# NTU-CompHydroMet-Lab/P2I-GAN-benchmark

Measured on AMD Instinct MI355X. Metric: train frames/sec (128x128x16), higher is better.
Workload: dtype f32

## Files before the change

p2i-gan-benchmark_amd/csrc/conv_x6c.hip:

```cpp
#include "conv_common.h"

namespace p2i {

#ifdef P2I_STAMP
extern __device__ unsigned long long* p2i_stamp_buf;
#define X6C_NOW(v) do { __builtin_amdgcn_sched_barrier(0); asm volatile("s_memtime %0\n\ts_waitcnt lgkmcnt(0)" : "=s"(v) :: "memory"); __builtin_amdgcn_sched_barrier(0); } while (0)
#define X6C_ACC(sum, t_prev) do { unsigned long long t_; X6C_NOW(t_); sum += t_ - t_prev; t_prev = t_; } while (0)
#else
#define X6C_NOW(v) do { } while (0)
#define X6C_ACC(sum, t_prev) do { } while (0)
#endif

typedef __bf16 bf16x8c __attribute__((ext_vector_type(8)));
typedef unsigned u32x4c __attribute__((ext_vector_type(4)));

__device__ __forceinline__ unsigned pack_hi16c(float lo_elem, float hi_elem) {
  return __builtin_amdgcn_perm(__float_as_uint(hi_elem), __float_as_uint(lo_elem), 0x07060302u);
}
__device__ __forceinline__ float trunc_bf16c(float v) { return __uint_as_float(__float_as_uint(v) & 0xFFFF0000u); }
__device__ __forceinline__ void split8c(const float (&v)[8], u32x4c& hi, u32x4c& mid, u32x4c& lo) {
#pragma unroll
  for (int j = 0; j < 4; ++j) {
    const float a = v[2 * j], b = v[2 * j + 1];
    hi[j] = pack_hi16c(a, b);
    const float ra = a - trunc_bf16c(a), rb = b - trunc_bf16c(b);
    mid[j] = pack_hi16c(ra, rb);
    const float sa = ra - trunc_bf16c(ra), sb = rb - trunc_bf16c(rb);
    lo[j] = pack_hi16c(sa, sb);
  }
}

template <class S, class I>
__device__ __forceinline__ void split8_store(const float* __restrict__ p, S stride, u32x4c* __restrict__ out, I total, I i) {
  float v[8];
#pragma unroll
  for (int q = 0; q < 8; ++q) v[q] = p[(S)q * stride];
  u32x4c h, mi, lo;
  split8c(v, h, mi, lo);
  out[i] = h;
  out[total + i] = mi;
  out[2 * total + i] = lo;
}

__global__ __launch_bounds__(256) void wsplit_kernel(const float* __restrict__ wp, u32x4c* __restrict__ wb, int ntaps, int Ck, int CmPad) {
  const int KCt = Ck >> 3;
  const int total = ntaps * KCt * CmPad;
  for (int i = blockIdx.x * 256 + threadIdx.x; i < total; i += gridDim.x * 256) {
    const int m = i % CmPad;
    const int r = i / CmPad;
    const int kc = r % KCt, tap = r / KCt;
    const float* p = wp + ((size_t)tap * Ck + kc * 8) * CmPad + m;
    split8_store(p, (size_t)CmPad, wb, total, i);
  }
}

struct WsplitBatch { const float* wp[24]; u32x4c* wb[24]; int ntaps[24], Ck[24], CmPad[24]; };
__global__ __launch_bounds__(256) void wsplit_batched_kernel(const WsplitBatch b) {
  const int L = blockIdx.y;
  const float* wp = b.wp[L];
  u32x4c* wb = b.wb[L];
  const int Ck = b.Ck[L], CmPad = b.CmPad[L], KCt = Ck >> 3;
  const int total = b.ntaps[L] * KCt * CmPad;
  for (int i = blockIdx.x * 256 + threadIdx.x; i < total; i += gridDim.x * 256) {
    const int m = i % CmPad;
    const int r = i / CmPad;
    const int kc = r % KCt, tap = r / KCt;
    const float* p = wp + ((size_t)tap * Ck + kc * 8) * CmPad + m;
    split8_store(p, (size_t)CmPad, wb, total, i);
  }
}

__global__ __launch_bounds__(256) void split_planes_kernel(const float* __restrict__ x, u32x4c* __restrict__ planes, int B, int KCt, long long P) {
  const long long total = (long long)B * KCt * P;
  for (long long i = blockIdx.x * 256ll + threadIdx.x; i < total; i += (long long)gridDim.x * 256) {
    const long long pix = i % P, r = i / P;
    const float* px = x + (r * 8) * P + pix;
    split8_store(px, P, planes, total, i);
  }
}

X6Ctx& x6_ctx() {
  static thread_local X6Ctx c{nullptr, 0};
  return c;
}

int x6_split_weights(const float* wp, uint16_t* wb, int ntaps, int Ck, int CmPad, hipStream_t s) {
  const int total = ntaps * (Ck >> 3) * CmPad;
  const int blocks = total > 0 ? (total + 255) / 256 : 1;
  P2I_LAUNCH(wsplit_kernel, dim3(blocks > 2048 ? 2048 : blocks), dim3(256), 0, s, wp, reinterpret_cast<u32x4c*>(wb), ntaps, Ck, CmPad);
  return launch_status();
}

struct X6cGeom {
  const float* src; float* dst; const uint16_t* wb; const float* bias; const float* res; const float* mask_y;
  unsigned wb_bytes;
  int act_epi, mask_act;
  int B, Ck, Cm, CmPad;
  int sH, sW, dT, dH, dW, nH, nW;
  int ljb, ljh, ljw, eH, eW, CSl, bH, bW, nth, ntw;
  unsigned mg_ew, mg_eh;
  int ntaps_w, ksplit;
  int sT, nT, mT, oT, pT, ns, sdt0, sdt1, sdt2, swt0, swt1, swt2;
  int tap_off[9];
  int tap_w[9];
  int fused_atomic;
  int stagger;
  int vec4_epi;
  const u32x4c* splanes;
  unsigned plane_units;
  int cons_prio;
};

__device__ constexpr int X6C_CLS[9] = {3, 3, 3, 3, 2, 2, 1, 1, 0};

template <int NW> struct X6cTile {
  static constexpr int MAXCSL = NW == 8 ? 384 : 256;
  static constexpr int NI = (2 * MAXCSL + 64 * NW - 1) / (64 * NW);
};

#define X6C_WAIT1(b) asm volatile("s_waitcnt vmcnt(%0)" ::"n"(b) : "memory")
#define X6C_WAIT2(b) if (n < (b) + 1) { X6C_WAIT1(b); } else { X6C_WAIT1((b) + 1); }
#define X6C_WAIT4(b) if (n < (b) + 2) { X6C_WAIT2(b) } else { X6C_WAIT2((b) + 2) }
#define X6C_WAIT8(b) if (n < (b) + 4) { X6C_WAIT4(b) } else { X6C_WAIT4((b) + 4) }
#define X6C_WAIT16(b) if (n < (b) + 8) { X6C_WAIT8(b) } else { X6C_WAIT8((b) + 8) }
#define X6C_WAIT32(b) if (n < (b) + 16) { X6C_WAIT16(b) } else { X6C_WAIT16((b) + 16) }
__device__ __forceinline__ void x6c_wait_vm(int n) {
  if (n < 0 || n > 62) n = 0;
  if (n < 32) { X6C_WAIT32(0) } else { X6C_WAIT32(32) }
}

template <int NW, int TM, bool FUSED = false, int TPS = 3>
__global__ __launch_bounds__(64 * NW) void patch_gemm_x6c_kernel(const X6cGeom g) {
  constexpr int NCLS = FUSED ? 4 : 1;
  constexpr int NSTG = 9 / TPS;
  static_assert(TPS == 3 || TPS == 9, "taps per stage");
  extern __shared__ __attribute__((aligned(16))) float smem[];
#ifdef P2I_STAMP
  unsigned long long st_entry, st_prev, st_wait = 0, st_bar = 0, st_issue = 0, st_mfma = 0, st_loop0;
  X6C_NOW(st_entry);
#endif
  constexpr int MB = 32 * TM, NTHR = 64 * NW, NI = X6cTile<NW>::NI;
  constexpr int RING = TPS == 9 ? 3 : (TM == 2 ? 4 : 6), LEAD = RING - 1;
  constexpr int WST = 6 * TPS * MB;
  constexpr int NWI = WST / 64;
  const int CSl = g.CSl;
  int* ptab = reinterpret_cast<int*>(smem);
  const int ptab_sz = (CSl + 3) & ~3;
  u32x4c* wbuf = reinterpret_cast<u32x4c*>(smem + ptab_sz);
  u32x4c* planes = wbuf + RING * WST;
  const int PST = 6 * CSl;

  const int tid = threadIdx.x, lane = tid & 63, wave = __builtin_amdgcn_readfirstlane(tid >> 6);
  const int l31 = lane & 31, lhi = lane >> 5;
  int tile = blockIdx.x;
  const int tw = tile % g.ntw; tile /= g.ntw;
  const int th = tile % g.nth;
  const int tb = tile / g.nth;
  const int j0b = tb << g.ljb, j0h = th << g.ljh, j0w = tw << g.ljw;
  const int o0 = blockIdx.y * MB;
  const int JWm = (1 << g.ljw) - 1, JHm = (1 << g.ljh) - 1;
  const int sHW = g.sH * g.sW;
  const int src_h0 = j0h + g.bH, src_w0 = j0w + g.bW;
  const int KCt = g.Ck >> 3;
  const int cps = g.Ck >> 4;
  const int cs = g.sT * sHW;
  const int nimg = g.B * g.nT;
  const int c0 = blockIdx.z * ((g.ns * cps) / g.ksplit);

  for (int e = tid; e < CSl; e += NTHR) {
    const int row = fast_div(e, g.mg_ew);
    const int ew = e - row * g.eW;
    const int jb = fast_div(row, g.mg_eh);
    const int eh = row - jb * g.eH;
    const int n = j0b + jb, h = src_h0 + eh, w = src_w0 + ew;
    const int b = n / g.nT, lt = n - b * g.nT;
    ptab[e] = (n < nimg && (unsigned)h < (unsigned)g.sH && (unsigned)w < (unsigned)g.sW) ? ((b * g.Ck) * g.sT + lt * g.mT) * sHW + h * g.sW + w : -1;
  }
  const int pix = wave * 32 + l31;
  const int pjw = pix & JWm, pjh = (pix >> g.ljw) & JHm, pjb = pix >> (g.ljw + g.ljh);
  const int lane_base = (pjb * g.eH + pjh) * g.eW + pjw + lhi * CSl;
  int toff[9];
#pragma unroll
  for (int t = 0; t < 9; ++t) toff[t] = g.tap_off[t];

  f32x16 acc[NCLS][TM];
#pragma unroll
  for (int q = 0; q < NCLS; ++q)
#pragma unroll
    for (int i = 0; i < TM; ++i)
#pragma unroll
      for (int r = 0; r < 16; ++r) acc[q][i][r] = 0.f;

  const v4i32 rs_w = make_rsrc(g.wb, g.wb_bytes);
  const unsigned wbuf_la = lds_base(smem) + 4u * ptab_sz;
  const int wl_m = TM == 2 ? lane : l31, wl_kg = TM == 2 ? 0 : lhi;
  const int wvoff = (o0 + wl_m < g.CmPad) ? (wl_kg * g.CmPad + wl_m) * 16 : -16;
  __syncthreads();

  int it_off[NI], it_dst[NI], it_f0[NI];
#pragma unroll
  for (int it = 0; it < NI; ++it) {
    const int item = it * NTHR + tid;
    const int kg = item >= CSl ? 1 : 0, e = item - kg * CSl;
    const bool in = item < 2 * CSl;
    const int po = in ? ptab[e] : -1;
    it_off[it] = po < 0 ? -1 : po + kg * 8 * cs;
    it_dst[it] = in ? kg * CSl + e : -1;
    const int jbi = fast_div(fast_div(in ? e : 0, g.mg_ew), g.mg_eh);
    it_f0[it] = ((j0b + jbi) % g.nT) * g.mT;
  }
  float pv[NI][8];
// ... 150 lines not shown
        if constexpr (TPS == 9) {
          if (more_c && (t == 4 || t == 6 || t == 7) && t == split_t) {
            x6c_wait_vm(nwb(sa));
            __builtin_amdgcn_sched_barrier(0);
            split_patch(planes + ((c + 1) & 1) * PST);
            __builtin_amdgcn_sched_barrier(0);
          }
        }
        load_tap(wsl, pb, TPS * b + t + 1, (t + 1) % 3);
        mfma_tap(t % 3, TPS * b + t);
        ilv();
        __builtin_amdgcn_sched_barrier(0);
      }
      if (TPS == 3 && late) { staging(); __builtin_amdgcn_sched_barrier(0); }
      X6C_ACC(st_mfma, st_prev);
      {
        int n = 0;
#pragma unroll
        for (int j = 2; j <= LEAD; ++j) n += nwb(s + j);
        if constexpr (TPS == 3) {
#pragma unroll
          for (int j = 0; j <= LEAD - 2; ++j) {
            const int bj = ((b - j) % 3 + 3) % 3;
            if (bj == 0 && s - j >= 0 && (s - j) / 3 + 1 < nch) n += NPL;
          }
        }
        x6c_wait_vm(n);
      }
      asm volatile("s_waitcnt lgkmcnt(0)" ::: "memory");
      X6C_ACC(st_wait, st_prev);
      __builtin_amdgcn_s_barrier();
      X6C_ACC(st_bar, st_prev);
      if (s + 1 < nst) load_tap(wlane + ((s + 1) % RING) * WST, b == NSTG - 1 ? pbn : pb, b == NSTG - 1 ? 0 : TPS * b + TPS, 0);
      mfma_tap(2, TPS * b + TPS - 1);
      ilv();
      __builtin_amdgcn_sched_barrier(0);
      X6C_ACC(st_mfma, st_prev);
    }
  }
#ifdef P2I_STAMP
  unsigned long long st_loop_end; X6C_NOW(st_loop_end);
#endif

  const int gw = j0w + pjw, gh = j0h + pjh, gn = j0b + pjb;
  const bool pvld = gn < nimg && gh < g.nH && gw < g.nW;
  const int dHW = g.dT * g.dH * g.dW;
  const int gb_ = gn / g.nT, glt = gn - gb_ * g.nT;
  if constexpr (FUSED) {
    const size_t pos0 = (size_t)gb_ * g.Cm * dHW + (size_t)(glt * g.oT + g.pT) * g.dH * g.dW + (size_t)(2 * gh) * g.dW + 2 * gw;
#pragma unroll
    for (int ph = 0; ph < 2; ++ph)
#pragma unroll
      for (int i = 0; i < TM; ++i)
        epilogue_pair16(acc[2 * ph][i], acc[2 * ph + 1][i], o0 + i * 32, lhi, g.Cm, pvld, pos0 + (size_t)ph * g.dW, (size_t)dHW,
                        (g.fused_atomic && blockIdx.z) ? nullptr : g.res, g.mask_y, g.mask_act, g.dst, g.fused_atomic != 0);
  } else {
    const size_t pos = (size_t)gb_ * g.Cm * dHW + (size_t)(glt * g.oT + g.pT) * g.dH * g.dW + (size_t)gh * g.dW + gw;
#pragma unroll
    for (int i = 0; i < TM; ++i)
      if (g.ksplit > 1)
        epilogue_tile16(acc[0][i], o0 + i * 32, lhi, g.Cm, pvld, pos, (size_t)dHW, blockIdx.z ? nullptr : g.bias, P2I_ACT_NONE,
                        blockIdx.z ? nullptr : g.res, g.mask_y, g.mask_act, g.dst, true);
      else
        epilogue_tile16(acc[0][i], o0 + i * 32, lhi, g.Cm, pvld, pos, (size_t)dHW, g.bias, g.act_epi, g.res, g.mask_y, g.mask_act, g.dst);
  }
#ifdef P2I_STAMP
  if (p2i_stamp_buf && lane == 0) {
    asm volatile("s_waitcnt vmcnt(0)" ::: "memory");
    unsigned long long st_x; X6C_NOW(st_x);
    unsigned long long* o = p2i_stamp_buf + ((size_t)(blockIdx.x + gridDim.x * blockIdx.y) * NW + wave) * 8;
    o[0] = st_wait; o[1] = st_bar; o[2] = st_issue; o[3] = st_mfma; o[4] = st_loop_end - st_loop0; o[5] = st_loop0; o[6] = st_loop0 - st_entry;
    o[7] = st_x - st_loop_end;
  }
#endif
}


template <int TM, int TPS, bool FUSED = false, bool EPI4 = false, int NPW = 4, int TN = 2, bool PRE = false>
__global__ __launch_bounds__(64 * (4 + NPW)) void patch_gemm_x6p_kernel(const X6cGeom g) {
  constexpr int NSTG = 9 / TPS;
  constexpr int NCLS = FUSED ? 4 : 1;
  static_assert(TPS == 3 || TPS == 9, "taps per stage");
  extern __shared__ __attribute__((aligned(16))) float smem[];
  constexpr int MB = 32 * TM, NCW = 4, NTHR = 64 * (NCW + NPW), NPT = 64 * NPW;
  constexpr int NI = (2 * (TN == 2 ? X6cTile<8>::MAXCSL : X6cTile<4>::MAXCSL) + NPT - 1) / NPT;
  constexpr int RING = TPS == 9 ? 3 : (TM == 2 ? 4 : 6), LEAD = RING - 1;
  constexpr int WST = 6 * TPS * MB, NWI = WST / 64;
  const int CSl = g.CSl;
  int* ptab = reinterpret_cast<int*>(smem);
  const int ptab_sz = (CSl + 3) & ~3;
  u32x4c* wbuf = reinterpret_cast<u32x4c*>(smem + ptab_sz);
  u32x4c* planes = wbuf + RING * WST;
  const int PST = 6 * CSl;

  const int tid = threadIdx.x, lane = tid & 63, wave = __builtin_amdgcn_readfirstlane(tid >> 6);
  const int l31 = lane & 31, lhi = lane >> 5;
  int tile = blockIdx.x;
  const int tw = tile % g.ntw; tile /= g.ntw;
  const int th = tile % g.nth;
  const int tb = tile / g.nth;
  const int j0b = tb << g.ljb, j0h = th << g.ljh, j0w = tw << g.ljw;
  const int o0 = blockIdx.y * MB;
  const int JWm = (1 << g.ljw) - 1, JHm = (1 << g.ljh) - 1;
  const int sHW = g.sH * g.sW;
  const int src_h0 = j0h + g.bH, src_w0 = j0w + g.bW;
  const int KCt = g.Ck >> 3;
  const int cps = g.Ck >> 4;
  const int cs = g.sT * sHW;
  const int nimg = g.B * g.nT;
  const int c0 = blockIdx.z * ((g.ns * cps) / g.ksplit);
  const int nch = (g.ns * cps) / g.ksplit;
  const int nst = NSTG * nch;

  for (int e = tid; e < CSl; e += NTHR) {
    const int row = fast_div(e, g.mg_ew);
    const int ew = e - row * g.eW;
    const int jb = fast_div(row, g.mg_eh);
    const int eh = row - jb * g.eH;
    const int n = j0b + jb, h = src_h0 + eh, w = src_w0 + ew;
    const int b = n / g.nT, lt = n - b * g.nT;
    ptab[e] = (n < nimg && (unsigned)h < (unsigned)g.sH && (unsigned)w < (unsigned)g.sW) ? ((b * (PRE ? KCt : g.Ck)) * g.sT + lt * g.mT) * sHW + h * g.sW + w : -1;
  }
  __syncthreads();

#ifdef P2I_STAMP
  unsigned long long st_a = 0, st_b = 0, st_c = 0, st_d = 0, st_e = 0, st_f = 0, st_t0, st_t1, st_l0 = 0, st_l1 = 0, st_entry;
  X6C_NOW(st_entry);
#endif
  if (wave >= NCW) {
    const int ptid = tid - 64 * NCW, pw = wave - NCW;
    const v4i32 rs_w = make_rsrc(g.wb, g.wb_bytes);
    const unsigned wbuf_la = lds_base(smem) + 4u * ptab_sz;
    const int wl_m = TM == 2 ? lane : l31, wl_kg = TM == 2 ? 0 : lhi;
    const int wvoff = (o0 + wl_m < g.CmPad) ? (wl_kg * g.CmPad + wl_m) * 16 : -16;
    int it_off[NI], it_dst[NI], it_f0[NI];
#pragma unroll
    for (int it = 0; it < NI; ++it) {
      const int item = it * NPT + ptid;
      const int kg = item >= CSl ? 1 : 0, e = item - kg * CSl;
      const bool in = item < 2 * CSl;
      const int po = in ? ptab[e] : -1;
      it_off[it] = po < 0 ? -1 : po + kg * (PRE ? 1 : 8) * cs;
      it_dst[it] = in ? kg * CSl + e : -1;
      const int jbi = fast_div(fast_div(in ? e : 0, g.mg_ew), g.mg_eh);
      it_f0[it] = ((j0b + jbi) % g.nT) * g.mT;
    }
    float pv[PRE ? 1 : NI][8];
    u32x4c pq[PRE ? NI : 1][3];
    bool pok[NI];
    auto load_patch = [&](int c) {
      if constexpr (PRE) {
        const int cg = c0 + c;
        const int j = cg >= 2 * cps ? 2 : (cg >= cps ? 1 : 0);
        const int dt = j == 2 ? g.sdt2 : (j == 1 ? g.sdt1 : g.sdt0);
        int voff[NI];
#pragma unroll
        for (int it = 0; it < NI; ++it) {
          pok[it] = it_off[it] >= 0 && (unsigned)(it_f0[it] + dt) < (unsigned)g.sT;
          voff[it] = pok[it] ? (it_off[it] + dt * sHW) * 16 : 0;
        }
#pragma unroll
        for (int p = 0; p < 3; ++p) {
          const u32x4c* sq = g.splanes + (size_t)p * g.plane_units + (size_t)(cg - j * cps) * 2 * cs;
          const unsigned long long sq_u = (unsigned long long)__builtin_amdgcn_readfirstlane((int)(unsigned)(unsigned long long)sq) & 0xffffffffull;
          const unsigned long long sq_hi = (unsigned long long)(unsigned)__builtin_amdgcn_readfirstlane((int)((unsigned long long)sq >> 32));
          const unsigned long long sbase = sq_u | (sq_hi << 32);
#pragma unroll
          for (int it = 0; it < NI; ++it) {
            if (it == 0) asm volatile("s_nop 4\n\tglobal_load_dwordx4 %0, %1, %2" : "=v"(pq[it][p]) : "v"(voff[it]), "s"(sbase) : "memory");
            else asm volatile("global_load_dwordx4 %0, %1, %2" : "=v"(pq[it][p]) : "v"(voff[it]), "s"(sbase) : "memory");
          }
        }
      } else {
      const int cg = c0 + c;
      const int j = cg >= 2 * cps ? 2 : (cg >= cps ? 1 : 0);
      const int dt = j == 2 ? g.sdt2 : (j == 1 ? g.sdt1 : g.sdt0);
      const float* sc = g.src + (size_t)(cg - j * cps) * 16 * cs;
      int voff[NI];
#pragma unroll
      for (int it = 0; it < NI; ++it) {
        pok[it] = it_off[it] >= 0 && (unsigned)(it_f0[it] + dt) < (unsigned)g.sT;
        voff[it] = pok[it] ? (it_off[it] + dt * sHW) * 4 : 0;
      }
#pragma unroll
      for (int q = 0; q < 8; ++q) {
        const float* sq = sc + (size_t)q * cs;
        const unsigned long long sq_u = (unsigned long long)__builtin_amdgcn_readfirstlane((int)(unsigned)(unsigned long long)sq) & 0xffffffffull;
        const unsigned long long sq_hi = (unsigned long long)(unsigned)__builtin_amdgcn_readfirstlane((int)((unsigned long long)sq >> 32));
        const unsigned long long sbase = sq_u | (sq_hi << 32);
#pragma unroll
        for (int it = 0; it < NI; ++it) {
          if (it == 0) asm volatile("s_nop 4\n\tglobal_load_dword %0, %1, %2" : "=v"(pv[it][q]) : "v"(voff[it]), "s"(sbase) : "memory");
          else asm volatile("global_load_dword %0, %1, %2" : "=v"(pv[it][q]) : "v"(voff[it]), "s"(sbase) : "memory");
        }
      }
      }
    };
    auto split_patch = [&](u32x4c* pb) {
      if constexpr (PRE) {
#pragma unroll
        for (int it = 0; it < NI; ++it)
#pragma unroll
          for (int p = 0; p < 3; ++p) asm volatile("" : "+v"(pq[it][p]));
        const u32x4c zero = {0u, 0u, 0u, 0u};
#pragma unroll
        for (int it = 0; it < NI; ++it) {
          if (it_dst[it] < 0) continue;
          pb[it_dst[it]] = pok[it] ? pq[it][0] : zero;
          pb[2 * CSl + it_dst[it]] = pok[it] ? pq[it][1] : zero;
          pb[4 * CSl + it_dst[it]] = pok[it] ? pq[it][2] : zero;
        }
      } else {
#pragma unroll
      for (int it = 0; it < NI; ++it)
#pragma unroll
        for (int q = 0; q < 8; ++q) asm volatile("" : "+v"(pv[it][q]));
#pragma unroll
      for (int it = 0; it < NI; ++it) {
        if (it_dst[it] < 0) continue;
        float v[8];
#pragma unroll
        for (int q = 0; q < 8; ++q) v[q] = pok[it] ? pv[it][q] : 0.f;
        u32x4c h, mi, lo;
        split8c(v, h, mi, lo);
        pb[it_dst[it]] = h;
        pb[2 * CSl + it_dst[it]] = mi;
        pb[4 * CSl + it_dst[it]] = lo;
      }
      }
    };
    constexpr int NWR = (NWI + NPW - 1) / NPW;
    int w_soff[NWR][NSTG];
    unsigned w_dst[NWR];
#pragma unroll
    for (int r = 0; r < NWR; ++r) {
      const int u = pw + NPW * r;
      const int pt = TM == 2 ? u >> 1 : u, kg = TM == 2 ? u & 1 : 0;
      const int p = pt / TPS, tl = pt % TPS;
#pragma unroll
      for (int b = 0; b < NSTG; ++b)
        w_soff[r][b] = u < NWI ? __builtin_amdgcn_readfirstlane((((p * g.ntaps_w + g.tap_w[TPS * b + tl]) * KCt + kg) * g.CmPad + o0) * 16) : 0;
      w_dst[r] = wbuf_la + 16u * (unsigned)(u * 64);
    }
    const int w_cstep = 2 * g.CmPad * 16;
    const int w_tstep = KCt * g.CmPad * 16;
    auto issue_w = [&](int c, int b, int sb) {
      const int cg = c0 + c;
      const int j = cg >= 2 * cps ? 2 : (cg >= cps ? 1 : 0);
      const int soff = (cg - j * cps) * w_cstep + (j == 2 ? g.swt2 : (j == 1 ? g.swt1 : g.swt0)) * w_tstep;
#pragma unroll
      for (int r = 0; r < NWR; ++r)
        if (pw + NPW * r < NWI) dma_b128(rs_w, w_dst[r] + 16u * (unsigned)(sb * WST), wvoff, w_soff[r][b] + soff);
    };
    const int nw_mine = (NWI / NPW) + (pw < NWI % NPW ? 1 : 0);
    constexpr int NPL = (PRE ? 3 : 8) * NI;
    auto nwb = [&](int st) { return (st >= LEAD && st < nst) ? nw_mine : 0; };
    load_patch(0);
    {
      int n = 0;
#pragma unroll
      for (int st = 0; st < LEAD; ++st) n += nwb(st);
      x6c_wait_vm(n);
      __builtin_amdgcn_sched_barrier(0);
      split_patch(planes);
      if constexpr (TPS == 9) {
        if (nch > 1) load_patch(1);
        x6c_wait_vm(n - nwb(0) + (nch > 1 ? NPL : 0));
      } else {
        x6c_wait_vm(n - nwb(0));
      }
    }
    asm volatile("s_waitcnt lgkmcnt(0)" ::: "memory");
    __builtin_amdgcn_s_barrier();
    int s = 0;
    for (int c = 0; c < nch; ++c) {
      const bool more_c = c + 1 < nch;
#pragma unroll
      for (int b = 0; b < NSTG; ++b, ++s) {
        const int sa = s + LEAD;
        if constexpr (TPS == 9) {
#ifdef P2I_STAMP
          X6C_NOW(st_t0);
          if (s == 0) st_l0 = st_t0;
#endif
          if (more_c) {
            x6c_wait_vm(s == 0 ? 0 : nwb(s - 1 + LEAD));
            X6C_ACC(st_a, st_t0);
            __builtin_amdgcn_sched_barrier(0);
            split_patch(planes + ((c + 1) & 1) * PST);
            __builtin_amdgcn_sched_barrier(0);
            X6C_ACC(st_b, st_t0);
            if (c + 2 < nch) load_patch(c + 2);
            X6C_ACC(st_e, st_t0);
          }
          if (sa < nst) issue_w(c + LEAD, 0, sa % RING);
          X6C_ACC(st_f, st_t0);
          x6c_wait_vm(nwb(s + 2) + ((more_c && c + 2 < nch) ? NPL : 0));
          X6C_ACC(st_c, st_t0);
        } else {
          if (b == 0 && more_c) load_patch(c + 1);
          if (sa < nst) issue_w(c + (b + LEAD) / NSTG, (b + LEAD) % NSTG, sa % RING);
          if (b == NSTG - 1 && more_c) {
            int n = 0;
#pragma unroll
            for (int j = 0; j < NSTG; ++j) n += nwb(sa - j);
            x6c_wait_vm(n);
            __builtin_amdgcn_sched_barrier(0);
            split_patch(planes + ((c + 1) & 1) * PST);
          }
          int n = 0;
#pragma unroll
          for (int j = 2; j <= LEAD; ++j) n += nwb(s + j);
#pragma unroll
          for (int j = 0; j <= LEAD - 2; ++j) {
            const int sj = s - j;
            if (sj >= 0 && sj % NSTG == 0 && sj / NSTG + 1 < nch) n += NPL;
          }
          x6c_wait_vm(n);
        }
        asm volatile("s_waitcnt lgkmcnt(0)" ::: "memory");
#ifdef P2I_STAMP
        X6C_NOW(st_t1);
#endif
        __builtin_amdgcn_s_barrier();
#ifdef P2I_STAMP
        X6C_ACC(st_d, st_t1);
        st_l1 = st_t1;
#endif
      }
    }
  }

  const bool producer = wave >= NCW;
  const int cw = wave & (NCW - 1);
  int lane_base[TN], pjw_[TN], pjh_[TN], pjb_[TN];
#pragma unroll
  for (int nb = 0; nb < TN; ++nb) {
    const int pix = cw * 32 * TN + nb * 32 + l31;
    pjw_[nb] = pix & JWm; pjh_[nb] = (pix >> g.ljw) & JHm; pjb_[nb] = pix >> (g.ljw + g.ljh);
    lane_base[nb] = (pjb_[nb] * g.eH + pjh_[nb]) * g.eW + pjw_[nb] + lhi * CSl;
  }
  int toff[9];
#pragma unroll
  for (int t = 0; t < 9; ++t) toff[t] = g.tap_off[t];
  f32x16 acc[NCLS][TM][TN];
#pragma unroll
  for (int q = 0; q < NCLS; ++q)
#pragma unroll
    for (int i = 0; i < TM; ++i)
#pragma unroll
      for (int nb = 0; nb < TN; ++nb)
#pragma unroll
        for (int r = 0; r < 16; ++r) acc[q][i][nb][r] = 0.f;
  constexpr int PA[6] = {2, 0, 1, 1, 0, 0};
  constexpr int PB[6] = {0, 2, 1, 0, 1, 0};
  u32x4c A[3][TM][3], Bv[3][TN][3];
  auto load_tap = [&](const u32x4c* wsl, const u32x4c* pbuf, int tap, int buf) {
    const int tl = tap % TPS;
    const int to = toff[tap];
#pragma unroll
    for (int p = 0; p < 3; ++p) {
#pragma unroll
      for (int i = 0; i < TM; ++i) A[buf][i][p] = wsl[((p * TPS + tl) * 2) * MB + 32 * i];
#pragma unroll
      for (int nb = 0; nb < TN; ++nb) Bv[buf][nb][p] = pbuf[lane_base[nb] + p * 2 * CSl + to];
    }
  };
  auto mfma_tap = [&](int buf, int slot) {
    const int cl = FUSED ? X6C_CLS[slot] : 0;
#pragma unroll
    for (int q = 0; q < 6; ++q)
#pragma unroll
      for (int i = 0; i < TM; ++i)
#pragma unroll
        for (int nb = 0; nb < TN; ++nb)
          acc[cl][i][nb] = __builtin_amdgcn_mfma_f32_32x32x16_bf16(__builtin_bit_cast(bf16x8c, A[buf][i][PA[q]]), __builtin_bit_cast(bf16x8c, Bv[buf][nb][PB[q]]),
                                                                   acc[cl][i][nb], 0, 0, 0);
  };
  auto ilv = [&]() {
    constexpr int NR = 3 * TM + 3 * TN, NM = 6 * TM * TN;
#pragma unroll
    for (int i = 0; i < NM; ++i) {
      __builtin_amdgcn_sched_group_barrier(0x008, 1, 0);
      if (i < NR) __builtin_amdgcn_sched_group_barrier(0x100, 1, 0);
    }
  };
  const int dHW = g.dT * g.dH * g.dW;
  const int mynb = (TN == 2 && producer) ? 1 : 0;
  const bool has_epi = wave < 2 * NCW;
  const bool split = FUSED ? g.fused_atomic != 0 : g.ksplit > 1;
  const float* const bias_q = (split && blockIdx.z) ? nullptr : g.bias;
  const float* const res_q = (split && blockIdx.z) ? nullptr : g.res;
  const bool blk1 = TN == 2 && producer;
  const int gw = j0w + (blk1 ? pjw_[TN - 1] : pjw_[0]), gh = j0h + (blk1 ? pjh_[TN - 1] : pjh_[0]), gn = j0b + (blk1 ? pjb_[TN - 1] : pjb_[0]);
  const bool pvld = gn < nimg && gh < g.nH && gw < g.nW;
  const int gb_ = gn / g.nT, glt = gn - gb_ * g.nT;
  const size_t img0 = (size_t)gb_ * g.Cm * dHW + (size_t)(glt * g.oT + g.pT) * g.dH * g.dW;
  const size_t pos0 = img0 + (size_t)(2 * gh) * g.dW + 2 * gw;
  const size_t pos = img0 + (size_t)gh * g.dW + gw;
  const int pg = cw * 32 * TN + mynb * 32 + 4 * (lane & 7);
  const int qw = pg & JWm, qh = (pg >> g.ljw) & JHm, qb = pg >> (g.ljw + g.ljh);
  const int hw = j0w + qw, hh = j0h + qh, hn = j0b + qb;
  const bool pv4 = hn < nimg && hh < g.nH && hw < g.nW;
  const int hb = hn / g.nT, hlt = hn - hb * g.nT;
  const size_t pos4 = (size_t)hb * g.Cm * dHW + (size_t)(hlt * g.oT + g.pT) * g.dH * g.dW + (size_t)hh * g.dW + hw;
  float* xch = reinterpret_cast<float*>(wbuf);
  float* tl = xch + 4 * NCLS * TM * 16 * 64 + wave * (32 * 36);
  EpiOps4p ops_p[FUSED ? 2 : 1];
  EpiOps4v ops_v[(!FUSED && EPI4) ? 2 : 1];
  EpiOps8 ops_t[(!FUSED && !EPI4) ? 2 : 1];
  auto fetch = [&](int slot, int k) {
    if constexpr (FUSED)
      epi_pair16_fetch(ops_p[slot], k & 3, o0 + ((k >> 2) % TM) * 32, lhi, g.Cm, pvld, pos0 + (size_t)(k / (4 * TM)) * g.dW, (size_t)dHW, res_q, g.mask_y);
    else if constexpr (EPI4)
      epi_tile16_v4_fetch(ops_v[slot], o0 + k * 32, lane, g.Cm, pos4, pv4, (size_t)dHW, bias_q, res_q, g.mask_y);
    else
      epi_tile16_fetch(ops_t[slot], k & 1, o0 + (k >> 1) * 32, lhi, g.Cm, pvld, pos, (size_t)dHW, bias_q, res_q, g.mask_y);
  };
  constexpr bool EARLY_C = !FUSED && TN == 1;
  const u32x4c* wlane = wbuf + lhi * MB + l31;
  if (!producer) {
    {
      const v4i32 rs_w = make_rsrc(g.wb, g.wb_bytes);
      const unsigned wbuf_la = lds_base(smem) + 4u * ptab_sz;
      const int wl_m = TM == 2 ? lane : l31, wl_kg = TM == 2 ? 0 : lhi;
      const int wvoff = (o0 + wl_m < g.CmPad) ? (wl_kg * g.CmPad + wl_m) * 16 : -16;
      const int w_cstep = 2 * g.CmPad * 16, w_tstep = KCt * g.CmPad * 16;
#pragma unroll
      for (int st = 0; st < LEAD; ++st) {
        if (st >= nst) break;
        const int cg = c0 + st / NSTG, b = st % NSTG;
        const int j = cg >= 2 * cps ? 2 : (cg >= cps ? 1 : 0);
        const int soff = (cg - j * cps) * w_cstep + (j == 2 ? g.swt2 : (j == 1 ? g.swt1 : g.swt0)) * w_tstep;
        for (int u = cw; u < NWI; u += NCW) {
          const int pt = TM == 2 ? u >> 1 : u, kg = TM == 2 ? u & 1 : 0;
          const int p = pt / TPS, tl = pt % TPS;
          const int so = (((p * g.ntaps_w + g.tap_w[TPS * b + tl]) * KCt + kg) * g.CmPad + o0) * 16 + soff;
          dma_b128(rs_w, wbuf_la + 16u * (unsigned)(u * 64 + (st % RING) * WST), wvoff, so);
        }
      }
      asm volatile("s_waitcnt vmcnt(0)" ::: "memory");
    }
    __builtin_amdgcn_s_barrier();
    if (g.cons_prio == 1) __builtin_amdgcn_s_setprio(1);
    else if (g.cons_prio == 2) __builtin_amdgcn_s_setprio(2);
    else if (g.cons_prio == 3) __builtin_amdgcn_s_setprio(3);
    load_tap(wlane, planes, 0, 0);
    int s = 0;
    for (int c = 0; c < nch; ++c) {
      const u32x4c* pb = planes + (c & 1) * PST;
      const u32x4c* pbn = planes + ((c + 1) & 1) * PST;
#pragma unroll
      for (int b = 0; b < NSTG; ++b, ++s) {
        const u32x4c* wsl = wlane + (s % RING) * WST;
        if constexpr (EARLY_C) { if (s + 1 == nst) fetch(0, 0); }
        __builtin_amdgcn_sched_barrier(0);
#pragma unroll
        for (int t = 0; t < TPS - 1; ++t) {
          load_tap(wsl, pb, TPS * b + t + 1, (t + 1) % 3);
          mfma_tap(t % 3, TPS * b + t);
          ilv();
          __builtin_amdgcn_sched_barrier(0);
        }
#ifdef P2I_STAMP
        X6C_NOW(st_t0);
        if (s == 0) st_l0 = st_t0;
#endif
        asm volatile("s_waitcnt lgkmcnt(0)" ::: "memory");
        X6C_ACC(st_a, st_t0);
        __builtin_amdgcn_s_barrier();
#ifdef P2I_STAMP
        X6C_ACC(st_d, st_t0);
        st_l1 = st_t0;
#endif
        if (s + 1 < nst) load_tap(wlane + ((s + 1) % RING) * WST, b == NSTG - 1 ? pbn : pb, b == NSTG - 1 ? 0 : TPS * b + TPS, 0);
        mfma_tap(2, TPS * b + TPS - 1);
        ilv();
        __builtin_amdgcn_sched_barrier(0);
      }
    }
  }
  if (!producer && g.cons_prio) __builtin_amdgcn_s_setprio(0);
  if (TN == 1 && producer) return;
  if (has_epi && !(EARLY_C && !producer)) fetch(0, 0);
  if constexpr (TN == 2) {
    if (!producer) {
#pragma unroll
      for (int q = 0; q < NCLS; ++q)
#pragma unroll
        for (int i = 0; i < TM; ++i)
#pragma unroll
          for (int r = 0; r < 16; ++r) xch[(((cw * NCLS + q) * TM + i) * 16 + r) * 64 + lane] = acc[q][i][1][r];
    }
    asm volatile("s_waitcnt lgkmcnt(0)" ::: "memory");
    __builtin_amdgcn_s_barrier();
    asm volatile("" ::: "memory");
    if (!has_epi) return;
    if (producer) {
#pragma unroll
      for (int q = 0; q < NCLS; ++q)
#pragma unroll
        for (int i = 0; i < TM; ++i)
#pragma unroll
          for (int r = 0; r < 16; ++r) acc[q][i][0][r] = xch[(((cw * NCLS + q) * TM + i) * 16 + r) * 64 + lane];
    }
  }
  if constexpr (FUSED) {
    auto finish = [&](int slot, int k) {
      const int ph = k / (4 * TM), i = (k >> 2) % TM;
      epi_pair16_finish(ops_p[slot], k & 3, acc[2 * ph][i][0], acc[2 * ph + 1][i][0], res_q, g.mask_y, g.mask_act, g.dst, split);
    };
    epilogue_pipelined<8 * TM>(fetch, finish, true);
  } else if constexpr (EPI4) {
    if (split) epilogue_pipelined<TM>(fetch, [&](int slot, int k) {
      epi_tile16_v4_finish(ops_v[slot], acc[0][k][0], tl, lane, P2I_ACT_NONE, res_q, g.mask_y, g.mask_act, g.dst, true); }, true);
    else epilogue_pipelined<TM>(fetch, [&](int slot, int k) {
      epi_tile16_v4_finish(ops_v[slot], acc[0][k][0], tl, lane, g.act_epi, g.res, g.mask_y, g.mask_act, g.dst, false); }, true);
  } else {
    if (split) epilogue_pipelined<2 * TM>(fetch, [&](int slot, int k) {
      epi_tile16_finish(ops_t[slot], k & 1, acc[0][k >> 1][0], bias_q, P2I_ACT_NONE, res_q, g.mask_y, g.mask_act, g.dst, true); }, true);
    else epilogue_pipelined<2 * TM>(fetch, [&](int slot, int k) {
      epi_tile16_finish(ops_t[slot], k & 1, acc[0][k >> 1][0], g.bias, g.act_epi, g.res, g.mask_y, g.mask_act, g.dst, false); }, true);
  }
#ifdef P2I_STAMP
  if (p2i_stamp_buf && lane == 0) {
    asm volatile("s_waitcnt vmcnt(0)" ::: "memory");
    unsigned long long st_end; X6C_NOW(st_end);
    unsigned long long* o = p2i_stamp_buf + ((size_t)(blockIdx.x + gridDim.x * blockIdx.y) * 8 + wave) * 8;
    o[0] = st_a; o[1] = st_d; o[2] = st_b; o[3] = st_c; o[4] = st_l1 - st_l0; o[5] = st_l0 - st_entry; o[6] = st_e; o[7] = st_end - st_l1;
  }
#endif
}

static bool x6c_on() { return P2I_ENV_ONCE("P2I_CONV_X6C", 1) != 0; }
static bool x6c_fused_on() { return P2I_ENV_ONCE("P2I_CONV_X6C_FUSED", 1) != 0; }
static int x6c_min_wg() { return env_int("P2I_X6C_MIN_WG", 200); }
static int x6c_min_wg_low() { return env_int("P2I_X6C_MIN_WG", env_int("P2I_X6C_MIN_WG_LOW", 64)); }
static int x6c_fused_min_wg() { return env_int("P2I_X6C_MIN_WG", 128); }
static int x6p_tn1() { return env_int("P2I_X6P_TN1", 1); }
static int x6c_forced() { return env_int("P2I_X6C_TILE", 0); }
static int x6c_stagger() { return env_int("P2I_X6C_STAGGER", 0); }
static int x6c_fused_ksplit() { return env_int("P2I_X6C_FUSED_KSPLIT", 0); }
static int x6p_npw() { return env_int("P2I_X6P_NPW", 8) == 4 ? 4 : 8; }
static int x6c_pc() { return env_int("P2I_X6C_PC", 1); }
static int x6c_tps1() { return env_int("P2I_X6C_TPS", 9) == 3 ? 3 : 9; }
static int x6p_prio() { return env_int("P2I_X6P_PRIO", 0); }

struct X6cVariant { int NW, TM; };
static const X6cVariant kX6cVariants[] = {{8, 2}, {8, 1}, {4, 1}};

struct X6cPick { int v, jb, jh, jw, csl, ksplit; long long wgs; };
static X6cPick x6c_pick(int B, int nH, int nW, int Cm, int Ck, bool linear_epi, int Ck_slice) {
  int forced = x6c_forced();
  const int min_wg = x6c_min_wg();
  const bool tn1_ok = x6c_pc() && Ck_slice >= 32;
  if (forced == 41 && !tn1_ok) forced = 81;
  const int ksplit_on = P2I_ENV_ONCE("P2I_X6C_KSPLIT", 1);
  static const int order_a[5][2] = {{0, 0}, {1, 0}, {2, 0}, {1, 1}, {0, 1}}, order_b[5][2] = {{0, 0}, {0, 1}, {1, 0}, {2, 0}, {1, 1}};
  X6cPick low{-1, 0, 0, 0, 0, 1, 0};
  for (int cand = 0; cand < 5; ++cand) {
      const int v = (ksplit_on == 2 ? order_b : order_a)[cand][0], pass = (ksplit_on == 2 ? order_b : order_a)[cand][1];
      const X6cVariant& t = kX6cVariants[v];
      if (v == 2 && (!tn1_ok || (forced ? forced != 41 : !x6p_tn1()))) continue;
      if (forced && forced != t.NW * 10 + t.TM) continue;
      if (t.TM == 2 && Cm <= 32 && !forced) continue;
      if (pass == 1 && ((ksplit_on != 2 && t.TM != 1) || !ksplit_on || !linear_epi || ((Ck >> 4) & 1) || forced)) continue;
      int jb, jt, jh, jw;
      pick_tile_dims(32 * t.NW, B, 1, nH, nW, jb, jt, jh, jw);
      const int csl = jb * (jh + 2) * (jw + 2);
      if (jt != 1 || csl > (t.NW == 8 ? X6cTile<8>::MAXCSL : X6cTile<4>::MAXCSL)) continue;
      const long long wgs = (long long)ceil_div(B, jb) * ceil_div(nH, jh) * ceil_div(nW, jw) * ceil_div(Cm, 32 * t.TM) * (pass + 1);
      if (wgs >= min_wg) return X6cPick{v, jb, jh, jw, csl, pass + 1, wgs};
      if (pass == 0 && !forced && wgs >= x6c_min_wg_low() && (low.v < 0 || wgs > low.wgs)) low = X6cPick{v, jb, jh, jw, csl, 1, wgs};
    }
  return low;
}

static X6cPick x6c_fused_pick(int nimg, int nH, int nW, int Cm, int chunks, bool may_split) {
  X6cPick pk{-1, 0, 0, 0, 0, 1, 0};
  int jt;
  pick_tile_dims(256, nimg, 1, nH, nW, pk.jb, jt, pk.jh, pk.jw);
  pk.csl = pk.jb * (pk.jh + 1) * (pk.jw + 1);
  if (jt != 1 || pk.csl > X6cTile<8>::MAXCSL) return pk;
  const long long tiles = (long long)ceil_div(nimg, pk.jb) * ceil_div(nH, pk.jh) * ceil_div(nW, pk.jw) * ceil_div(Cm, 32);
  const bool can_split = x6c_fused_ksplit() && may_split && (chunks & 1) == 0;
  const int min_wg = x6c_fused_min_wg();
  if (tiles < min_wg && !(can_split && 2 * tiles >= min_wg)) return pk;
  pk.ksplit = tiles < min_wg ? 2 : 1;
  pk.wgs = tiles * pk.ksplit;
  pk.v = 1;
  return pk;
}

bool x6c_would_take(const p2i_conv_desc* d, bool dgrad, int act_epi) {
  const bool on = x6c_on();
  (void)act_epi;
  if (on && dgrad && d->sh == 2 && d->sw == 2 && d->st == 1 && d->kh == 3 && d->kw == 3 && d->ph == 1 && d->pw == 1 &&
      ((d->kt == 1 && d->pt == 0) || (d->kt == 3 && d->pt == 1)) && (d->Cout & 15) == 0 && d->Cout >= 16 && !(d->Hi & 1) && !(d->Wi & 1))
    return x6c_fused_on() && x6c_fused_pick(d->B * d->Ti, d->Hi / 2, d->Wi / 2, d->Cin, d->kt * (d->Cout >> 4), true).v >= 0;
  if (!on || d->kh != 3 || d->kw != 3 || d->sh != 1 || d->sw != 1 || d->ph != 1 || d->pw != 1) return false;
  const bool flat = d->kt == 1 && d->st == 1 && d->pt == 0;
  const bool vol = d->kt == 3 && d->pt == 1 && d->st <= 2;
  if (!flat && !vol) return false;
  const int Ck = dgrad ? d->Cout : d->Cin, Cm = dgrad ? d->Cin : d->Cout;
  const int nH = dgrad ? d->Hi : d->Ho, nW = dgrad ? d->Wi : d->Wo;
  if ((Ck & 15) != 0 || Ck < 16) return false;
  const int nT = dgrad ? d->Ti / d->st : d->To;
  if (nT < 1) return false;
  const int ns = flat ? 1 : (dgrad && d->st == 2 ? 1 : 3);
  const bool whole = !dgrad || d->st == 1;
  return x6c_pick(d->B * nT, nH, nW, Cm, ns * Ck, whole, Ck).v >= 0;
}

__global__ __launch_bounds__(256) void x6c_post_act_kernel(float* __restrict__ y, const float* __restrict__ res, long long n4, int act) {
// ... 225 lines not shown
```

Baseline: 12130.

## Overlap x6p prologue: prefetch weights early, drop ptab barrier, per-item patch split

For TM==2 variants of the producer/consumer patch GEMM, consumer waves issue the first weight-stage DMAs at kernel entry, before any tile index math. Producers compute patch offsets directly instead of going through a shared ptab table and a block-wide __syncthreads. They also issue the first patch loads with hand-written global_load_dword and split each item into bf16 planes as soon as its loads land. A kernarg warm-up loads one dword per cache line of the argument block. The aim is to shorten the kernel prologue and hide global-load latency, at the cost of more register pressure and inline-asm fragility. Profiling stamps are extended as well.

```diff
diff --git a/p2i-gan-benchmark_amd/csrc/conv_x6c.hip b/p2i-gan-benchmark_amd/csrc/conv_x6c.hip
--- a/p2i-gan-benchmark_amd/csrc/conv_x6c.hip
+++ b/p2i-gan-benchmark_amd/csrc/conv_x6c.hip
@@ -6,9 +6,11 @@
 extern __device__ unsigned long long* p2i_stamp_buf;
 #define X6C_NOW(v) do { __builtin_amdgcn_sched_barrier(0); asm volatile("s_memtime %0\n\ts_waitcnt lgkmcnt(0)" : "=s"(v) :: "memory"); __builtin_amdgcn_sched_barrier(0); } while (0)
 #define X6C_ACC(sum, t_prev) do { unsigned long long t_; X6C_NOW(t_); sum += t_ - t_prev; t_prev = t_; } while (0)
+#define X6C_PRO(i) X6C_ACC(st_p[i], st_pt)
 #else
 #define X6C_NOW(v) do { } while (0)
 #define X6C_ACC(sum, t_prev) do { } while (0)
+#define X6C_PRO(i) do { } while (0)
 #endif
 
 typedef __bf16 bf16x8c __attribute__((ext_vector_type(8)));
@@ -127,6 +129,15 @@
 __device__ __forceinline__ void x6c_wait_vm(int n) {
   if (n < 0 || n > 62) n = 0;
   if (n < 32) { X6C_WAIT32(0) } else { X6C_WAIT32(32) }
+}
+
+__device__ __forceinline__ void x6c_warm_kernarg() {
+  static_assert(sizeof(X6cGeom) == 0x138, "one dword per 64-byte line of the argument, and its last dword");
+  const void* ka = (const void*)__builtin_amdgcn_kernarg_segment_ptr();
+  unsigned d0, d1, d2, d3, d4, d5;
+  asm volatile("s_load_dword %0, %6, 0x0\n\ts_load_dword %1, %6, 0x40\n\ts_load_dword %2, %6, 0x80\n\ts_load_dword %3, %6, 0xc0\n\t"
+               "s_load_dword %4, %6, 0x100\n\ts_load_dword %5, %6, 0x134\n\ts_waitcnt lgkmcnt(0)"
+               : "=&s"(d0), "=&s"(d1), "=&s"(d2), "=&s"(d3), "=&s"(d4), "=&s"(d5) : "s"(ka) : "memory");
 }
 
 template <int NW, int TM, bool FUSED = false, int TPS = 3>
@@ -443,10 +454,17 @@
   constexpr int NCLS = FUSED ? 4 : 1;
   static_assert(TPS == 3 || TPS == 9, "taps per stage");
   extern __shared__ __attribute__((aligned(16))) float smem[];
-  constexpr int MB = 32 * TM, NCW = 4, NTHR = 64 * (NCW + NPW), NPT = 64 * NPW;
+  constexpr int MB = 32 * TM, NCW = 4, NPT = 64 * NPW;
   constexpr int NI = (2 * (TN == 2 ? X6cTile<8>::MAXCSL : X6cTile<4>::MAXCSL) + NPT - 1) / NPT;
   constexpr int RING = TPS == 9 ? 3 : (TM == 2 ? 4 : 6), LEAD = RING - 1;
   constexpr int WST = 6 * TPS * MB, NWI = WST / 64;
+#ifdef P2I_STAMP
+  unsigned long long st_p[7] = {0, 0, 0, 0, 0, 0, 0}, st_pt;
+  X6C_NOW(st_pt);
+#endif
+  constexpr bool PIF = TM == 2;
+  if constexpr (PIF) x6c_warm_kernarg();
+  X6C_PRO(0);
   const int CSl = g.CSl;
   int* ptab = reinterpret_cast<int*>(smem);
   const int ptab_sz = (CSl + 3) & ~3;
@@ -456,6 +474,41 @@
 
   const int tid = threadIdx.x, lane = tid & 63, wave = __builtin_amdgcn_readfirstlane(tid >> 6);
   const int l31 = lane & 31, lhi = lane >> 5;
+  if (PIF && wave < NCW) {
+    const int o0 = blockIdx.y * MB;
+    const int KCt = g.Ck >> 3, cps = g.Ck >> 4;
+    const int nch = (g.ns * cps) / g.ksplit, c0 = blockIdx.z * nch, nst = NSTG * nch;
+    const v4i32 rs_w = make_rsrc(g.wb, g.wb_bytes);
+    const unsigned wbuf_la = lds_base(smem) + 4u * ptab_sz;
+    const int wl_m = TM == 2 ? lane : l31, wl_kg = TM == 2 ? 0 : lhi;
+    const int wvoff = (o0 + wl_m < g.CmPad) ? (wl_kg * g.CmPad + wl_m) * 16 : -16;
+    const int w_cstep = 2 * g.CmPad * 16, w_tstep = KCt * g.CmPad * 16;
+    constexpr int NWC = (NWI + NCW - 1) / NCW;
+    int w_so[LEAD][NWC];
+#pragma unroll
+    for (int st = 0; st < LEAD; ++st) {
+      const int cg = c0 + st / NSTG, b = st % NSTG;
+      const int j = cg >= 2 * cps ? 2 : (cg >= cps ? 1 : 0);
+      const int soff = (cg - j * cps) * w_cstep + (j == 2 ? g.swt2 : (j == 1 ? g.swt1 : g.swt0)) * w_tstep;
+#pragma unroll
+      for (int k = 0; k < NWC; ++k) {
+        const int u = wave + NCW * k < NWI ? wave + NCW * k : NWI - 1;
+        const int pt = TM == 2 ? u >> 1 : u, kg = TM == 2 ? u & 1 : 0;
+        const int p = pt / TPS, tl = pt % TPS;
+        w_so[st][k] = (((p * g.ntaps_w + g.tap_w[TPS * b + tl]) * KCt + kg) * g.CmPad + o0) * 16 + soff;
+      }
+    }
+#pragma unroll
+    for (int st = 0; st < LEAD; ++st) {
+      if (st >= nst) break;
+#pragma unroll
+      for (int k = 0; k < NWC; ++k) {
+        const int u = wave + NCW * k;
+        if (u < NWI) dma_b128(rs_w, wbuf_la + 16u * (unsigned)(u * 64 + (st % RING) * WST), wvoff, w_so[st][k]);
+      }
+    }
+    X6C_PRO(2);
+  }
   int tile = blockIdx.x;
   const int tw = tile % g.ntw; tile /= g.ntw;
   const int th = tile % g.nth;
@@ -473,20 +526,38 @@
   const int nch = (g.ns * cps) / g.ksplit;
   const int nst = NSTG * nch;
 
-  for (int e = tid; e < CSl; e += NTHR) {
-    const int row = fast_div(e, g.mg_ew);
-    const int ew = e - row * g.eW;
-    const int jb = fast_div(row, g.mg_eh);
-    const int eh = row - jb * g.eH;
-    const int n = j0b + jb, h = src_h0 + eh, w = src_w0 + ew;
-    const int b = n / g.nT, lt = n - b * g.nT;
-    ptab[e] = (n < nimg && (unsigned)h < (unsigned)g.sH && (unsigned)w < (unsigned)g.sW) ? ((b * (PRE ? KCt : g.Ck)) * g.sT + lt * g.mT) * sHW + h * g.sW + w : -1;
-  }
-  __syncthreads();
+  if constexpr (!PIF) {
+    constexpr int NTHR = 64 * (NCW + NPW);
+    for (int e = tid; e < CSl; e += NTHR) {
+      const int row = fast_div(e, g.mg_ew);
+      const int ew = e - row * g.eW;
+      const int jb = fast_div(row, g.mg_eh);
+      const int eh = row - jb * g.eH;
+      const int n = j0b + jb, h = src_h0 + eh, w = src_w0 + ew;
+      const int b = n / g.nT, lt = n - b * g.nT;
+      ptab[e] = (n < nimg && (unsigned)h < (unsigned)g.sH && (unsigned)w < (unsigned)g.sW) ? ((b * (PRE ? KCt : g.Ck)) * g.sT + lt * g.mT) * sHW + h * g.sW + w : -1;
+    }
+    __syncthreads();
+    X6C_PRO(0);
+  }
 
 #ifdef P2I_STAMP
   unsigned long long st_a = 0, st_b = 0, st_c = 0, st_d = 0, st_e = 0, st_f = 0, st_t0, st_t1, st_l0 = 0, st_l1 = 0, st_entry;
   X6C_NOW(st_entry);
+  auto stamp_out = [&]() {
+    if (p2i_stamp_buf && lane == 0) {
+      asm volatile("s_waitcnt vmcnt(0)" ::: "memory");
+      unsigned long long st_end; X6C_NOW(st_end);
+      unsigned long long* o = p2i_stamp_buf + ((size_t)(blockIdx.x + gridDim.x * blockIdx.y) * 12 + wave) * 16;
+      o[0] = st_a; o[1] = st_d; o[2] = st_b; o[3] = st_c; o[4] = st_l1 - st_l0; o[5] = st_l0 - st_entry; o[6] = st_e; o[7] = st_end - st_l1;
+#pragma unroll
+      for (int i = 0; i < 7; ++i) o[8 + i] = st_p[i];
+      o[15] = NCW + NPW;
+    }
+  };
+#define X6C_STAMP_OUT() stamp_out()
+#else
+#define X6C_STAMP_OUT() do { } while (0)
 #endif
   if (wave >= NCW) {
     const int ptid = tid - 64 * NCW, pw = wave - NCW;
@@ -500,11 +571,24 @@
       const int item = it * NPT + ptid;
       const int kg = item >= CSl ? 1 : 0, e = item - kg * CSl;
       const bool in = item < 2 * CSl;
-      const int po = in ? ptab[e] : -1;
-      it_off[it] = po < 0 ? -1 : po + kg * (PRE ? 1 : 8) * cs;
+      if constexpr (!PIF) {
+        const int po = in ? ptab[e] : -1;
+        it_off[it] = po < 0 ? -1 : po + kg * (PRE ? 1 : 8) * cs;
+        it_dst[it] = in ? kg * CSl + e : -1;
+        const int jbi = fast_div(fast_div(in ? e : 0, g.mg_ew), g.mg_eh);
+        it_f0[it] = ((j0b + jbi) % g.nT) * g.mT;
+        continue;
+      }
+      const int row = fast_div(in ? e : 0, g.mg_ew);
+      const int ew = (in ? e : 0) - row * g.eW;
+      const int jb = fast_div(row, g.mg_eh);
+      const int eh = row - jb * g.eH;
+      const int n = j0b + jb, h = src_h0 + eh, w = src_w0 + ew;
+      const int b = n / g.nT, lt = n - b * g.nT;
+      const bool ok = in && n < nimg && (unsigned)h < (unsigned)g.sH && (unsigned)w < (unsigned)g.sW;
+      it_off[it] = ok ? ((b * (PRE ? KCt : g.Ck)) * g.sT + lt * g.mT) * sHW + h * g.sW + w + kg * (PRE ? 1 : 8) * cs : -1;
       it_dst[it] = in ? kg * CSl + e : -1;
-      const int jbi = fast_div(fast_div(in ? e : 0, g.mg_ew), g.mg_eh);
-      it_f0[it] = ((j0b + jbi) % g.nT) * g.mT;
+      it_f0[it] = lt * g.mT;
     }
     float pv[PRE ? 1 : NI][8];
     u32x4c pq[PRE ? NI : 1][3];
@@ -557,6 +641,44 @@
       }
       }
     };
+    auto load_patch_items = [&](int c) {
+      const int cg = c0 + c;
+      const int j = cg >= 2 * cps ? 2 : (cg >= cps ? 1 : 0);
+      const int dt = j == 2 ? g.sdt2 : (j == 1 ? g.sdt1 : g.sdt0);
+      const float* sc = g.src + (size_t)(cg - j * cps) * 16 * cs;
+      int voff[NI];
+#pragma unroll
+      for (int it = 0; it < NI; ++it) {
+        pok[it] = it_off[it] >= 0 && (unsigned)(it_f0[it] + dt) < (unsigned)g.sT;
+        voff[it] = pok[it] ? (it_off[it] + dt * sHW) * 4 : 0;
+      }
+      unsigned long long sbase[8];
+#pragma unroll
+      for (int q = 0; q < 8; ++q) {
+        const float* sq = sc + (size_t)q * cs;
+        const unsigned long long sq_u = (unsigned long long)__builtin_amdgcn_readfirstlane((int)(unsigned)(unsigned long long)sq) & 0xffffffffull;
+        const unsigned long long sq_hi = (unsigned long long)(unsigned)__builtin_amdgcn_readfirstlane((int)((unsigned long long)sq >> 32));
+        sbase[q] = sq_u | (sq_hi << 32);
+      }
+#pragma unroll
+      for (int it = 0; it < NI; ++it)
+#pragma unroll
+        for (int q = 0; q < 8; ++q)
+          asm volatile("s_nop 4\n\tglobal_load_dword %0, %1, %2" : "=v"(pv[PRE ? 0 : it][q]) : "v"(voff[it]), "s"(sbase[q]) : "memory");
+    };
+    auto split_item = [&](u32x4c* pb, int it) {
+#pragma unroll
+      for (int q = 0; q < 8; ++q) asm volatile("" : "+v"(pv[PRE ? 0 : it][q]));
+      if (it_dst[it] < 0) return;
+      float v[8];
+#pragma unroll
+      for (int q = 0; q < 8; ++q) v[q] = pok[it] ? pv[PRE ? 0 : it][q] : 0.f;
+      u32x4c h, mi, lo;
+      split8c(v, h, mi, lo);
+      pb[it_dst[it]] = h;
+      pb[2 * CSl + it_dst[it]] = mi;
+      pb[4 * CSl + it_dst[it]] = lo;
+    };
     auto split_patch = [&](u32x4c* pb) {
       if constexpr (PRE) {
 #pragma unroll
@@ -590,17 +712,23 @@
       }
       }
     };
+    if constexpr (PIF) {
+      X6C_PRO(1);
+      load_patch_items(0);
+      X6C_PRO(2);
+    }
     constexpr int NWR = (NWI + NPW - 1) / NPW;
     int w_soff[NWR][NSTG];
     unsigned w_dst[NWR];
 #pragma unroll
     for (int r = 0; r < NWR; ++r) {
       const int u = pw + NPW * r;
-      const int pt = TM == 2 ? u >> 1 : u, kg = TM == 2 ? u & 1 : 0;
+      const int uc = (!PIF || u < NWI) ? u : NWI - 1;
+      const int pt = TM == 2 ? uc >> 1 : uc, kg = TM == 2 ? uc & 1 : 0;
       const int p = pt / TPS, tl = pt % TPS;
 #pragma unroll
       for (int b = 0; b < NSTG; ++b)
-        w_soff[r][b] = u < NWI ? __builtin_amdgcn_readfirstlane((((p * g.ntaps_w + g.tap_w[TPS * b + tl]) * KCt + kg) * g.CmPad + o0) * 16) : 0;
+        w_soff[r][b] = (PIF || u < NWI) ? __builtin_amdgcn_readfirstlane((((p * g.ntaps_w + g.tap_w[TPS * b + tl]) * KCt + kg) * g.CmPad + o0) * 16) : 0;
       w_dst[r] = wbuf_la + 16u * (unsigned)(u * 64);
     }
     const int w_cstep = 2 * g.CmPad * 16;
@@ -616,14 +744,32 @@
     const int nw_mine = (NWI / NPW) + (pw < NWI % NPW ? 1 : 0);
     constexpr int NPL = (PRE ? 3 : 8) * NI;
     auto nwb = [&](int st) { return (st >= LEAD && st < nst) ? nw_mine : 0; };
-    load_patch(0);
+    if constexpr (!PIF) {
+      X6C_PRO(1);
+      load_patch(0);
+      X6C_PRO(2);
+    }
     {
       int n = 0;
 #pragma unroll
       for (int st = 0; st < LEAD; ++st) n += nwb(st);
-      x6c_wait_vm(n);
-      __builtin_amdgcn_sched_barrier(0);
-      split_patch(planes);
+      if constexpr (!PIF) {
+        x6c_wait_vm(n);
+        X6C_PRO(3);
+        __builtin_amdgcn_sched_barrier(0);
+        split_patch(planes);
+        X6C_PRO(4);
+      } else {
+#pragma unroll
+        for (int it = 0; it < NI; ++it) {
+          x6c_wait_vm(n + 8 * (NI - 1 - it));
+          X6C_PRO(3);
+          __builtin_amdgcn_sched_barrier(0);
+          split_item(planes, it);
+          __builtin_amdgcn_sched_barrier(0);
+          X6C_PRO(4);
+        }
+      }
       if constexpr (TPS == 9) {
         if (nch > 1) load_patch(1);
         x6c_wait_vm(n - nwb(0) + (nch > 1 ? NPL : 0));
@@ -632,7 +778,9 @@
       }
     }
     asm volatile("s_waitcnt lgkmcnt(0)" ::: "memory");
+    X6C_PRO(5);
     __builtin_amdgcn_s_barrier();
+    X6C_PRO(6);
     int s = 0;
     for (int c = 0; c < nch; ++c) {
       const bool more_c = c + 1 < nch;
@@ -781,7 +929,8 @@
   constexpr bool EARLY_C = !FUSED && TN == 1;
   const u32x4c* wlane = wbuf + lhi * MB + l31;
   if (!producer) {
-    {
+    X6C_PRO(1);
+    if constexpr (!PIF) {
       const v4i32 rs_w = make_rsrc(g.wb, g.wb_bytes);
       const unsigned wbuf_la = lds_base(smem) + 4u * ptab_sz;
       const int wl_m = TM == 2 ? lane : l31, wl_kg = TM == 2 ? 0 : lhi;
@@ -800,9 +949,12 @@
           dma_b128(rs_w, wbuf_la + 16u * (unsigned)(u * 64 + (st % RING) * WST), wvoff, so);
         }
       }
-      asm volatile("s_waitcnt vmcnt(0)" ::: "memory");
-    }
+      X6C_PRO(2);
+    }
+    asm volatile("s_waitcnt vmcnt(0)" ::: "memory");
+    X6C_PRO(3);
     __builtin_amdgcn_s_barrier();
+    X6C_PRO(4);
     if (g.cons_prio == 1) __builtin_amdgcn_s_setprio(1);
     else if (g.cons_prio == 2) __builtin_amdgcn_s_setprio(2);
     else if (g.cons_prio == 3) __builtin_amdgcn_s_setprio(3);
@@ -842,7 +994,7 @@
     }
   }
   if (!producer && g.cons_prio) __builtin_amdgcn_s_setprio(0);
-  if (TN == 1 && producer) return;
+  if (TN == 1 && producer) { X6C_STAMP_OUT(); return; }
   if (has_epi && !(EARLY_C && !producer)) fetch(0, 0);
   if constexpr (TN == 2) {
     if (!producer) {
@@ -856,7 +1008,7 @@
     asm volatile("s_waitcnt lgkmcnt(0)" ::: "memory");
     __builtin_amdgcn_s_barrier();
     asm volatile("" ::: "memory");
-    if (!has_epi) return;
+    if (!has_epi) { X6C_STAMP_OUT(); return; }
     if (producer) {
 #pragma unroll
       for (int q = 0; q < NCLS; ++q)
@@ -883,14 +1035,8 @@
     else epilogue_pipelined<2 * TM>(fetch, [&](int slot, int k) {
       epi_tile16_finish(ops_t[slot], k & 1, acc[0][k >> 1][0], g.bias, g.act_epi, g.res, g.mask_y, g.mask_act, g.dst, false); }, true);
   }
-#ifdef P2I_STAMP
-  if (p2i_stamp_buf && lane == 0) {
-    asm volatile("s_waitcnt vmcnt(0)" ::: "memory");
-    unsigned long long st_end; X6C_NOW(st_end);
-    unsigned long long* o = p2i_stamp_buf + ((size_t)(blockIdx.x + gridDim.x * blockIdx.y) * 8 + wave) * 8;
-    o[0] = st_a; o[1] = st_d; o[2] = st_b; o[3] = st_c; o[4] = st_l1 - st_l0; o[5] = st_l0 - st_entry; o[6] = st_e; o[7] = st_end - st_l1;
-  }
-#endif
+  X6C_STAMP_OUT();
+#undef X6C_STAMP_OUT
 }
 
 static bool x6c_on() { return P2I_ENV_ONCE("P2I_CONV_X6C", 1) != 0; }
```

After: 12200, median of 6. No clear change (+0.6%).
